# fanliaoooo/xuanpolicy

Measured on AMD Instinct MI355X. Metric: env-steps/sec at num_envs=4096, horizon=128; GAE kernel HBM GB/s vs peak, higher is better.
Workload: dtype f32; 1 GPU; PPO-Clip SynthBox(obs=17,act=6) num_envs=4096/GPU horizon=128, ppo/mujoco.yaml (n_epoch 16, n_minibatch 8, nets [256] LeakyReLU); num_envs_per_gpu=4096, horizon=128, global_envs=4096, minibatch=65536, parallelism=dp1 (one env shard, no collective)

## Files before the change

include/xuanpolicy_amd.h:

```cpp
#ifndef XUANPOLICY_AMD_H
#define XUANPOLICY_AMD_H

#include <stdint.h>

#ifdef __cplusplus
extern "C" {
#endif

typedef struct ihipStream_t *xpa_stream_t;

#define XPA_ABI_VERSION 4
#define XPA_COLSUM_TICKET_INTS 4096

typedef struct {
    int32_t ptr;
    uint32_t step;
    int32_t reserved[2];
} xpa_cursor_t;

enum { XPA_ALGO_PPO = 0, XPA_ALGO_A2C = 1 };
enum { XPA_DIST_GAUSSIAN = 0, XPA_DIST_CATEGORICAL = 1 };

enum {
    XPA_OUT_ACTOR_LOSS = 0,
// ... 332 lines not shown

int xpa_head_gemm_s3_actor(int algo, int dist, int act, int64_t batch, int64_t act_dim, int64_t hidden, const float *x,
                           int64_t ldx, const float *w_hidden, const float *b_hidden, int64_t ld_dz, const float *w,
                           const float *b, float slope, const float *logstd, const int64_t *idx, int64_t n_rows,
                           const float *act_buf, const float *old_logp, const float *adv, const double *adv_partials,
                           int64_t n_adv_partials, float clip_range, float ent_coef, float *dz, float *partial_dw,
                           float *partial_db_hidden, float *partial_db_out, float *loss_partials, int64_t loss_width,
                           xpa_stream_t stream);
int xpa_head_gemm_s3_critic(int act, int64_t batch, int64_t hidden, const float *x, int64_t ldx,
                            const float *w_hidden, const float *b_hidden, int64_t ld_dz, const float *w, const float *b,
                            float slope, const int64_t *idx, int64_t n_rows, const float *ret, float vf_coef, float *dz,
                            float *partial_dw, float *partial_db_hidden, float *partial_db_out, float *loss_partials,
                            int64_t loss_width, xpa_stream_t stream);

int xpa_head_gemm_s3p_actor(int algo, int dist, int act, int64_t batch, int64_t act_dim, int64_t hidden, const float *x,
                            int64_t ldx, const float *w_hidden_split, const float *b_hidden, int64_t ld_dz,
                            const float *w, const float *b, float slope, const float *logstd, const int64_t *idx,
                            int64_t n_rows, const float *act_buf, const float *old_logp, const float *adv,
                            const double *adv_partials, int64_t n_adv_partials, float clip_range, float ent_coef,
                            float *dz, float *partial_dw, float *partial_db_hidden, float *partial_db_out,
                            float *loss_partials, int64_t loss_width, xpa_stream_t stream);
int xpa_head_gemm_s3p_critic(int act, int64_t batch, int64_t hidden, const float *x, int64_t ldx,
                             const float *w_hidden_split, const float *b_hidden, int64_t ld_dz, const float *w,
                             const float *b, float slope, const int64_t *idx, int64_t n_rows, const float *ret,
                             float vf_coef, float *dz, float *partial_dw, float *partial_db_hidden,
                             float *partial_db_out, float *loss_partials, int64_t loss_width, xpa_stream_t stream);
int xpa_head_gemm_s3q_actor(int algo, int dist, int act, int64_t batch, int64_t act_dim, int64_t hidden, const float *x,
                            int64_t ldx, const float *w_hidden_split, const float *b_hidden, int64_t ld_dz,
                            const float *w, const float *b, float slope, const float *logstd, const int64_t *idx,
                            int64_t n_rows, const float *act_buf, const float *old_logp, const float *adv,
                            const double *adv_partials, int64_t n_adv_partials, float clip_range, float ent_coef,
                            float *dz, float *partial_dw, float *partial_db_hidden, float *partial_db_out,
                            float *loss_partials, int64_t loss_width, xpa_stream_t stream);
int xpa_head_gemm_s3q_critic(int act, int64_t batch, int64_t hidden, const float *x, int64_t ldx,
                             const float *w_hidden_split, const float *b_hidden, int64_t ld_dz, const float *w,
                             const float *b, float slope, const int64_t *idx, int64_t n_rows, const float *ret,
                             float vf_coef, float *dz, float *partial_dw, float *partial_db_hidden,
                             float *partial_db_out, float *loss_partials, int64_t loss_width, xpa_stream_t stream);

int xpa_head_gemm_trunk_actor(int algo, int dist, int act, int64_t batch, int64_t act_dim, int64_t hidden,
                              const float *x_rows, int64_t ld_rows, int64_t d_in, const float *w_in, const float *b_in,
                              float slope_in, float *h_out, int64_t ld_h, const float *w_hidden, const float *b_hidden,
                              int64_t ld_dz, const float *w, const float *b, float slope, const float *logstd,
                              const int64_t *idx, int64_t n_rows, const float *act_buf, const float *old_logp,
                              const float *adv, const double *adv_partials, int64_t n_adv_partials, float clip_range,
                              float ent_coef, float *dz, float *partial_dw, float *partial_db_hidden,
                              float *partial_db_out, float *loss_partials, int64_t loss_width, xpa_stream_t stream);
int xpa_head_gemm_trunk_critic(int act, int64_t batch, int64_t hidden, const float *x_rows, int64_t ld_rows,
                               int64_t d_in, const float *w_in, const float *b_in, float slope_in, float *h_out,
                               int64_t ld_h, const float *w_hidden, const float *b_hidden, int64_t ld_dz, const float *w,
                               const float *b, float slope, const int64_t *idx, int64_t n_rows, const float *ret,
                               float vf_coef, float *dz, float *partial_dw, float *partial_db_hidden,
                               float *partial_db_out, float *loss_partials, int64_t loss_width, xpa_stream_t stream);

int64_t xpa_s3_split_bytes(int64_t k, int64_t n);
int xpa_s3_probe(int mask);
int xpa_s3_split_b(const float *b, int64_t k, int64_t n, int64_t sk, int64_t sn, void *out, xpa_stream_t stream);
int xpa_s3_split_batch(int n_mat, const float *const *b, const int64_t *k, const int64_t *sk, const int64_t *sn,
                       void *const *out, xpa_stream_t stream);
int xpa_s3_gemm(const float *a, int64_t lda, const void *b_split, float *c, int64_t ldc, int64_t m, int64_t k, int64_t n,
                xpa_stream_t stream);
int xpa_s3_gemm_group(int n, const float *const *a, const void *const *b_split, float *const *c, int64_t lda,
                      int64_t ldc, int64_t m, int64_t k, xpa_stream_t stream);
int64_t xpa_s3_gemm_group_act_num_partials(int n, int64_t m);
int xpa_s3_gemm_group_act(int n, const float *const *a, const void *const *b_split, float *const *c,
                          const float *const *y, int64_t lda, int64_t ldc, int64_t m, int64_t k, int act, float slope,
                          int64_t channels, float *bias_partial, xpa_stream_t stream);
int64_t xpa_s3_wgrad_num_slices(int64_t rows, int64_t m);
int64_t xpa_s3_gemm_trunk_bwd_num_partials(int64_t rows);
int xpa_s3_gemm_trunk_bwd(const float *dz, int64_t ldz, const void *b_split, int64_t k, const float *h, int64_t ldh,
                          const float *x, int64_t ldx, int64_t rows, int64_t d_in, int act, float slope,
                          float *partial_dw, float *partial_db, xpa_stream_t stream);
int xpa_s3_wgrad(const float *a, int64_t lda, const float *b, int64_t ldb, int64_t rows, int64_t m, int64_t n,
                 int64_t slices, float *out, xpa_stream_t stream);
int xpa_s3_gemm_trunk_bwd_sign(const float *dz, int64_t ldz, const void *b_split, int64_t k, const unsigned *h_sign,
                               const float *x, int64_t ldx, int64_t rows, int64_t d_in, int act, float slope,
                               float *partial_dw, float *partial_db, xpa_stream_t stream);
int xpa_head_gemm_s3q_critic_mask(int act, int64_t batch, int64_t hidden, const float *x, int64_t ldx,
                                  const float *w_hidden_split, const float *b_hidden, int64_t ld_dz, const float *w,
                                  const float *b, float slope, const int64_t *idx, int64_t n_rows, const float *ret,
                                  float vf_coef, float *dz, float *partial_dw, float *partial_db_hidden,
                                  float *partial_db_out, float *loss_partials, int64_t loss_width, xpa_stream_t stream,
                                  unsigned *mask, float *dv);
int xpa_s3_split_batch_scaled(int n_mat, const float *const *b, const int64_t *k, const int64_t *sk, const int64_t *sn,
                              void *const *out, const float *const *rs_w, const float *rs_a, const int64_t *rs_from,
                              float *cs_out, float cs_slope, xpa_stream_t stream);
int xpa_s3_gemm_trunk_bwd_crit(const float *dz_a, int64_t ldz, const void *b_split, int64_t k_a, int64_t k_c,
                               const unsigned *crit_mask, const float *crit_dv, const float *crit_cs,
                               const unsigned *h_sign, const float *x, int64_t ldx, int64_t rows, int64_t d_in, int act,
                               float slope, float *partial_dw, float *partial_db, xpa_stream_t stream);
int xpa_s3_wgrad_pair_slices(int64_t rows, int64_t *sa, int64_t *sc, int64_t *per_a, int64_t *per_c);
int xpa_s3_wgrad_pair_tune(int sa_target);
int xpa_s3_wgrad_pair(const float *dz_a, int64_t lda, const float *h, int64_t ldb, int64_t rows,
                      const unsigned *crit_mask, const float *crit_dv, const float *crit_wc, float crit_slope,
                      int64_t sa, int64_t per_a, int64_t sc, int64_t per_c, float *out_a, float *out_c,
                      xpa_stream_t stream);
int xpa_rollout_post_deferred_norm_rms(
    int64_t n_envs, int64_t horizon, const float *rew, const uint8_t *term, const uint8_t *trunc, const float *final_obs,
    int64_t ld_final, const float *slot_src, int64_t ld_slot, int64_t obs_dim, float *obs_mean, float *obs_var,
    double *obs_count, float obs_clip, float *boot_norm, int64_t ld_norm, float *slot_obs, int32_t *slot_t,
    int64_t n_slots, int32_t *overflow, xpa_cursor_t *cursor, float *ret_mean, float *ret_var, double *ret_count,
    float *returns, float *buf_rew, float *buf_term, uint8_t *buf_closed, float *buf_boot, float gamma,
    int mask_returns, int use_rewnorm, float rew_range, int atari_lifeloss, double *partials, uint32_t *ticket,
    const float *rms_x, int64_t rms_ld, double *rms_part, xpa_stream_t stream);
int xpa_s3_gemm_bias_act_rows(const float *a, int64_t lda, const int64_t *ridx, const void *b_split, float *c,
                              int64_t ldc, int64_t m, int64_t k, const float *bias, int act, float slope,
                              unsigned *sign_out, xpa_stream_t stream);
int xpa_s3_wgrad_rows(const float *a, int64_t lda, const int64_t *aidx, const float *b, int64_t ldb, int64_t rows,
                      int64_t m, int64_t n, int64_t slices, float *out, xpa_stream_t stream);
int xpa_s3_wgrad_padded(const float *a, int64_t lda, const float *b, int64_t ldb, int64_t rows, int64_t m, int64_t n,
                        int64_t slices, float *out, xpa_stream_t stream);
int xpa_s3_gemm_rows_pair(const float *a, int64_t lda, const void *b0_split, const void *b1_split, const float *bias,
                          float *c, int64_t ldc, int64_t m, xpa_stream_t stream);
int xpa_gather_minibatch_pitched(const int64_t *idx, int64_t batch, int64_t n_rows, const void *obs,
                                 int64_t obs_row_bytes, void *obs_out, int64_t out_row_bytes, const float *adv,
                                 double *adv_partials, int32_t *err, xpa_stream_t stream);
int xpa_s3_split_batch_padded(int n_mat, const float *const *b, const int64_t *k, const int64_t *kv, const int64_t *sk,
                              const int64_t *sn, void *const *out, xpa_stream_t stream);
int xpa_s3_gemm_bias_act(const float *a, int64_t lda, const void *b_split, float *c, int64_t ldc, int64_t m, int64_t k,
                         const float *bias, int act, float slope, unsigned *sign_out, xpa_stream_t stream);
int xpa_s3_gemm_trunk_bwd_dz(const float *dz, int64_t ldz, const void *b_split, int64_t k, const unsigned *h_sign,
                             int64_t rows, int act, float slope, float *dz_out, int64_t ld_out, float *partial_db,
                             xpa_stream_t stream);
int xpa_s3_gemm_trunk_bwd_crit_dz(const float *dz_a, int64_t ldz, const void *b_split, int64_t k_a, int64_t k_c,
                                  const unsigned *crit_mask, const float *crit_dv, const float *crit_cs,
                                  const unsigned *h_sign, int64_t rows, int act, float slope, float *dz_out,
                                  int64_t ld_out, float *partial_db, xpa_stream_t stream);
int xpa_colsum_finalize_batch_map(int n_segs, const float *const *partials, const int64_t *n_partials,
                                  const int64_t *cols, float *const *outs, const int64_t *tmap, double *sq,
                                  int32_t *ticket, int algo, int dist, int64_t batch, int64_t act_dim,
                                  const float *loss_partials, int64_t n_loss_partials, float vf_coef, float ent_coef,
                                  float *scalars, float *d_logstd, xpa_stream_t stream);
int xpa_head_gemm_s3r_actor(int algo, int dist, int act, int64_t batch, int64_t act_dim, int64_t hidden,
                            const float *x_rows, int64_t ld_rows, int64_t d_in, const float *w_in, const float *b_in,
                            float slope_in, float *h_out, int64_t ld_h, unsigned *h_sign, const void *w_hidden,
                            const float *b_hidden, int64_t ld_dz, const float *w, const float *b, float slope,
                            const float *logstd, const int64_t *idx, int64_t n_rows, const float *act_buf,
                            const float *old_logp, const float *adv, const double *adv_partials,
                            int64_t n_adv_partials, float clip_range, float ent_coef, float *dz, float *partial_dw,
                            float *partial_db_hidden, float *partial_db_out, float *loss_partials, int64_t loss_width,
                            xpa_stream_t stream);
int xpa_head_gemm_s3r_critic(int act, int64_t batch, int64_t hidden, const float *x_rows, int64_t ld_rows,
                             int64_t d_in, const float *w_in, const float *b_in, float slope_in, const void *w_hidden,
                             const float *b_hidden, int64_t ld_dz, const float *w, const float *b, float slope,
                             const int64_t *idx, int64_t n_rows, const float *ret, float vf_coef, float *dz,
                             float *partial_dw, float *partial_db_hidden, float *partial_db_out, float *loss_partials,
                             int64_t loss_width, xpa_stream_t stream);

int xpa_per_store(double *sum_tree, double *min_tree, const double *max_priority, int64_t n_envs,
                  int64_t capacity, int64_t ptr, double alpha, xpa_stream_t stream);
int xpa_per_update_priorities(double *sum_tree, double *min_tree, double *max_priority, int *scratch,
                              int64_t n_envs, int64_t capacity, int64_t size, const int64_t *idx,
                              const float *priorities, int64_t batch_per_env, double alpha, int *err,
                              xpa_stream_t stream);
int xpa_per_sample(const double *sum_tree, const double *min_tree, int64_t n_envs, int64_t capacity, int64_t size,
                   int64_t batch_per_env, int64_t n_size, const double *uniforms, uint32_t seed, uint32_t counter,
                   double beta, int wrap_uint8, int64_t *steps, int64_t *flat_index, double *weights, int32_t *err,
                   xpa_stream_t stream);

int xpa_store_column(const void *src, int64_t n, int64_t row_bytes, void *dst, int64_t horizon,
                     const xpa_cursor_t *cursor, xpa_stream_t stream);

int xpa_synthatari_step(int64_t n_envs, int64_t n_actions, const float *act_in, int64_t ld_act, uint32_t seed,
                        int32_t max_episode_steps, uint8_t *stack, uint8_t *final_obs, float *rew, uint8_t *term,
                        uint8_t *trunc, int32_t *ep_step, int32_t *ep_index, int32_t *lives, int32_t *paddle,
                        float *ep_score, float *ep_last_score, int32_t *ep_last_len, int32_t *err,
// ... 120 lines not shown
```

xuanpolicy_amd/csrc/sgemm3.hip:

```cpp
#include "xpa_common.h"
#include "s3_split.h"

namespace {

typedef xpa_f32x16 f32x16;
typedef xpa_bf16x8 bf16x8;
typedef __attribute__((address_space(3))) char lds_char_t;

constexpr int kN = 256;
constexpr int kKC = 16;
constexpr int kBImg = 3 * kN * kKC * 2;
template <int W>
struct S3Geom {
    static constexpr int kRows = 32 * W;
    static constexpr int kAImg = kRows * kKC * 4;
    static constexpr int kStage = kAImg + kBImg;
    static constexpr int kPer = kBImg / 1024 / W;
    static constexpr int kDma = 2 + kPer;
    static_assert(kBImg % (1024 * W) == 0, "B image splits evenly over the waves");
};

__device__ __forceinline__ void glds16(const void *g, unsigned lds_wave_base) {
    asm volatile("s_mov_b32 m0, %1\n\ts_nop 0\n\tglobal_load_lds_dwordx4 %0, off" ::"v"(g), "s"(lds_wave_base)
                 : "memory", "m0");
// ... 1148 lines not shown
        if (t < 256) {
            s_dv[t] = r0 + t < M ? cdv[r0 + t] : 0.f;
            s_cs[t] = ccs[t];
        }
    }
    __syncthreads();
    f32x16 acc[8];
#pragma unroll
    for (int cb = 0; cb < 8; ++cb)
#pragma unroll
        for (int r = 0; r < 16; ++r) acc[cb][r] = 0.f;
    const int N = nca + ncc;
    auto chunk_of = [&](int i) { return i < ncc ? nca + i : i - ncc; };
    auto issue_i = [&](int i) {
        const unsigned st = base + (i % 3) * G::kStage;
        const int c = chunk_of(i);
        const int rr = lane >> 2, p = lane & 3;
        if (i >= ncc) {
            const int q = p ^ ((rr >> 2) & 3);
#pragma unroll
            for (int k = 0; k < 2; ++k) {
                int64_t row = r0 + wave * 32 + k * 16 + rr;
                row = row < M ? row : M - 1;
                glds16(a + row * lda + c * kKC + 4 * q, st + (unsigned)((wave * 32 + k * 16) * kKC * 4));
            }
        }
        const char *bsrc = reinterpret_cast<const char *>(bs) + (int64_t)c * kBImg;
#pragma unroll
        for (int j = 0; j < G::kPer; ++j) {
            const int piece = wave * G::kPer + j;
            glds16(bsrc + piece * 1024 + lane * 16, st + (unsigned)(G::kAImg + piece * 1024));
        }
    };
    auto wait_i = [&](int i) {
        if (i + 1 >= N) asm volatile("s_waitcnt vmcnt(0)\n\ts_barrier" ::: "memory");
        else if (i + 1 >= ncc) asm volatile("s_waitcnt vmcnt(%0)\n\ts_barrier" ::"n"(G::kDma) : "memory");
        else asm volatile("s_waitcnt vmcnt(%0)\n\ts_barrier" ::"n"(G::kPer) : "memory");
    };
    issue_i(0);
    if (N > 1) issue_i(1);
    const int hh = lane >> 5, i32 = lane & 31;
    const unsigned *mrow = s_mask + (wave * 32 + i32) * kCMaskStride;
#pragma unroll 1
    for (int i = 0; i < ncc; ++i) {
        wait_i(i);
        if (i + 2 < N) issue_i(i + 2);
        const unsigned wbits = mrow[i >> 1] >> (16 * (i & 1) + 4 * hh);
        unsigned pk[4];
#pragma unroll
        for (int pj = 0; pj < 4; ++pj) {
            const int j0 = 2 * pj, j1 = 2 * pj + 1;
            const int b0 = j0 < 4 ? j0 : j0 + 4, b1 = j1 < 4 ? j1 : j1 + 4;
            pk[pj] = (((wbits >> b0) & 1u) * 0x3F80u) | ((((wbits >> b1) & 1u) * 0x3F80u) << 16);
        }
        const bf16x8 am = __builtin_bit_cast(bf16x8, make_uint4(pk[0], pk[1], pk[2], pk[3]));
        const bf16x8 *bimg = reinterpret_cast<const bf16x8 *>(lds + (i % 3) * G::kStage + G::kAImg) + lane;
#pragma unroll
        for (int cb = 0; cb < 8; ++cb) {
            acc[cb] = __builtin_amdgcn_mfma_f32_32x32x16_bf16(am, bimg[(16 + cb) * 64], acc[cb], 0, 0, 0);
            acc[cb] = __builtin_amdgcn_mfma_f32_32x32x16_bf16(am, bimg[(8 + cb) * 64], acc[cb], 0, 0, 0);
            acc[cb] = __builtin_amdgcn_mfma_f32_32x32x16_bf16(am, bimg[cb * 64], acc[cb], 0, 0, 0);
        }
    }
    {
        const int col = lane & 31;
#pragma unroll
        for (int r = 0; r < 16; ++r) {
            const float dvr = s_dv[wave * 32 + (r & 3) + 8 * (r >> 2) + 4 * hh];
#pragma unroll
            for (int cb = 0; cb < 8; ++cb) acc[cb][r] = dvr * (acc[cb][r] + s_cs[cb * 32 + col]);
        }
    }
#pragma unroll 1
    for (int i = ncc; i < N; ++i) {
        wait_i(i);
        if (i + 2 < N) issue_i(i + 2);
        chunk<8, 0>(lds + (i % 3) * G::kStage, acc, lane, wave);
    }
    __syncthreads();
    tb_epilogue<ACT, true, DZ>(acc, lds, r0, M, t, lane, wave, nullptr, 0, x, ldx, din, slope, p_dw, p_db, hsign,
                               dz_out, ld_out);
}

constexpr int kWgM = 128;
constexpr int kWgKC = 32;
constexpr int kWgAImg = 3 * 4 * 2 * 1024;
constexpr int kWgBImg = 3 * 8 * 2 * 1024;
constexpr int kWgStage = kWgAImg + kWgBImg;

struct WgUnits {
    float a[8], b0[8], b1[8];
};

__device__ __forceinline__ void wg_load(WgUnits &u, const float *__restrict__ A, int64_t lda, const float *__restrict__ B,
                                        int64_t ldb, int64_t k0, int64_t kend, int ma, int sa, int ha, int nb, int sb) {
#pragma unroll
    for (int j = 0; j < 8; ++j) {
        const int64_t ra = k0 + 16 * sa + kmap(ha, j);
        const int64_t rb0 = k0 + 16 * sb + kmap(0, j), rb1 = k0 + 16 * sb + kmap(1, j);
        const float va = A[min(ra, kend - 1) * lda + ma];
        const float v0 = B[min(rb0, kend - 1) * ldb + nb], v1 = B[min(rb1, kend - 1) * ldb + nb];
        u.a[j] = ra < kend ? va : 0.f;
        u.b0[j] = rb0 < kend ? v0 : 0.f;
        u.b1[j] = rb1 < kend ? v1 : 0.f;
    }
}

__device__ __forceinline__ void wg_put(char *st, const float (&v)[8], int off) {
    bf16x8 h, m, l;
    xpa_split8(make_float4(v[0], v[1], v[2], v[3]), make_float4(v[4], v[5], v[6], v[7]), h, m, l);
    *reinterpret_cast<bf16x8 *>(st + off) = h;
    *reinterpret_cast<bf16x8 *>(st + off + 8 * 1024 * ((off < kWgAImg) ? 1 : 2)) = m;
    *reinterpret_cast<bf16x8 *>(st + off + 16 * 1024 * ((off < kWgAImg) ? 1 : 2)) = l;
}

__device__ __forceinline__ void wg_store(char *st, const WgUnits &u, int ml, int sa, int ha, int nb, int sb) {
    wg_put(st, u.a, (((ml >> 5) * 2 + sa) * 64 + ha * 32 + (ml & 31)) * 16);
    wg_put(st, u.b0, kWgAImg + (((nb >> 5) * 2 + sb) * 64 + (nb & 31)) * 16);
    wg_put(st, u.b1, kWgAImg + (((nb >> 5) * 2 + sb) * 64 + 32 + (nb & 31)) * 16);
}

template <int PROBE>
__device__ __forceinline__ void wg_chunk(const char *st, f32x16 (&acc)[2][2], int lane, int wm, int wn) {
#pragma unroll
    for (int s = 0; s < 2; ++s) {
        bf16x8 ah[2], am[2], al[2], bh[2], bm[2], bl[2];
#pragma unroll
        for (int i = 0; i < 2; ++i) {
            const bf16x8 *pa = reinterpret_cast<const bf16x8 *>(st) + ((2 * wm + i) * 2 + s) * 64 + lane;
            ah[i] = pa[0];
            am[i] = pa[8 * 64];
            al[i] = pa[16 * 64];
            const bf16x8 *pb = reinterpret_cast<const bf16x8 *>(st + kWgAImg) + ((2 * wn + i) * 2 + s) * 64 + lane;
            bh[i] = pb[0];
            bm[i] = pb[16 * 64];
            bl[i] = pb[32 * 64];
        }
        if constexpr ((PROBE & 5) != 0) {
#pragma unroll
            for (int i = 0; i < 2; ++i)
#pragma unroll
                for (int j = 0; j < 2; ++j) {
                    if constexpr ((PROBE & 1) != 0)
                        asm volatile("" ::"v"(ah[i]), "v"(am[i]), "v"(al[i]), "v"(bh[j]), "v"(bm[j]), "v"(bl[j]));
                    else acc[i][j] = __builtin_amdgcn_mfma_f32_32x32x16_bf16(ah[i], bh[j], acc[i][j], 0, 0, 0);
                    if constexpr ((PROBE & 1) == 0) asm volatile("" ::"v"(am[i]), "v"(al[i]), "v"(bm[j]), "v"(bl[j]));
                }
            continue;
        }
#pragma unroll
        for (int i = 0; i < 2; ++i)
#pragma unroll
            for (int j = 0; j < 2; ++j) acc[i][j] = xpa_mfma_s3(ah[i], am[i], al[i], bh[j], bm[j], bl[j], acc[i][j]);
    }
}

template <int PROBE>
__global__ __launch_bounds__(512, 1) void s3_wgrad_kernel(const float *__restrict__ A, int64_t lda,
                                                          const float *__restrict__ B, int64_t ldb, int64_t rows,
                                                          int64_t M, int slices, int64_t slice_rows,
                                                          float *__restrict__ out) {
    __shared__ __attribute__((aligned(16))) char lds[2 * kWgStage];
    const int mtiles = (int)(M / kWgM);
    const int nblk = slices * mtiles;
    int L = blockIdx.x;
    if (nblk % 8 == 0) L = (blockIdx.x & 7) * (nblk >> 3) + (blockIdx.x >> 3);
// ... 910 lines not shown
                                          const float *crit_cs, const unsigned *h_sign, int64_t rows, int act,
                                          float slope, float *dz_out, int64_t ld_out, float *partial_db,
                                          xpa_stream_t stream) {
    if (!dz_a || !b_split || !crit_mask || !crit_dv || !crit_cs || !h_sign || !dz_out || !partial_db || rows <= 0 ||
        k_a <= 0 || k_c <= 0 || k_a % kKC != 0 || k_c % kKC != 0 || k_c > 256 || ldz < k_a || (ldz & 3) ||
        (reinterpret_cast<uintptr_t>(dz_a) & 15) || (reinterpret_cast<uintptr_t>(h_sign) & 15) ||
        (reinterpret_cast<uintptr_t>(crit_mask) & 15) || ld_out < kN || act < 0 || act > 1 ||
        (k_a + k_c) / kKC > (1 << 20))
        return (int)hipErrorInvalidValue;
    const dim3 grid((unsigned)xpa_s3_gemm_trunk_bwd_num_partials(rows)), block(512);
    const __bf16 *bs = static_cast<const __bf16 *>(b_split);
    const int nca = (int)(k_a / kKC), ncc = (int)(k_c / kKC);
    if (act == 0)
        s3_trunk_bwd_crit_kernel<0, true><<<grid, block, 0, stream>>>(dz_a, ldz, bs, rows, nca, ncc, crit_mask,
                                                                       crit_dv, crit_cs, nullptr, 0, 0, slope, nullptr,
                                                                       partial_db, h_sign, dz_out, ld_out);
    else
        s3_trunk_bwd_crit_kernel<1, true><<<grid, block, 0, stream>>>(dz_a, ldz, bs, rows, nca, ncc, crit_mask,
                                                                       crit_dv, crit_cs, nullptr, 0, 0, slope, nullptr,
                                                                       partial_db, h_sign, dz_out, ld_out);
    return xpa_launch_status();
}

namespace {
int gemm_bias_act_impl(const float *a, int64_t lda, const int64_t *ridx, const void *b_split, float *c, int64_t ldc,
                       int64_t m, int64_t k, const float *bias, int act, float slope, unsigned *sign_out,
                       xpa_stream_t stream);
}

XPA_API int xpa_s3_gemm_bias_act(const float *a, int64_t lda, const void *b_split, float *c, int64_t ldc, int64_t m,
                                 int64_t k, const float *bias, int act, float slope, unsigned *sign_out,
                                 xpa_stream_t stream) {
    if (lda < k) return (int)hipErrorInvalidValue;
    return gemm_bias_act_impl(a, lda, nullptr, b_split, c, ldc, m, k, bias, act, slope, sign_out, stream);
}

XPA_API int xpa_s3_gemm_bias_act_rows(const float *a, int64_t lda, const int64_t *ridx, const void *b_split, float *c,
                                      int64_t ldc, int64_t m, int64_t k, const float *bias, int act, float slope,
                                      unsigned *sign_out, xpa_stream_t stream) {
    if (!ridx || lda < 4 || k > lda + kKC) return (int)hipErrorInvalidValue;
    return gemm_bias_act_impl(a, lda, ridx, b_split, c, ldc, m, k, bias, act, slope, sign_out, stream);
}

namespace {
int gemm_bias_act_impl(const float *a, int64_t lda, const int64_t *ridx, const void *b_split, float *c, int64_t ldc,
                       int64_t m, int64_t k, const float *bias, int act, float slope, unsigned *sign_out,
                       xpa_stream_t stream) {
    if (!a || !b_split || !c || !bias || m <= 0 || k <= 0 || k % kKC != 0 || ldc < kN ||
        (reinterpret_cast<uintptr_t>(a) & 15) || (lda & 3) || act < 0 || act > 2 || (sign_out && act == 2) ||
        (reinterpret_cast<uintptr_t>(sign_out) & 15) || k / kKC > (1 << 20))
        return (int)hipErrorInvalidValue;
    const __bf16 *bs = static_cast<const __bf16 *>(b_split);
    const int nch = (int)(k / kKC);
    const dim3 grid((unsigned)((m + 255) / 256)), block(512);
    unsigned char *sg = reinterpret_cast<unsigned char *>(sign_out);
    if (act == 0)
        s3_gemm_kernel<8, 3, 0, 0, 1><<<grid, block, 0, stream>>>(a, lda, bs, c, ldc, m, nch, bias, slope, sg, ridx);
    else if (act == 1)
        s3_gemm_kernel<8, 3, 0, 0, 2><<<grid, block, 0, stream>>>(a, lda, bs, c, ldc, m, nch, bias, slope, sg, ridx);
    else
        s3_gemm_kernel<8, 3, 0, 0, 3><<<grid, block, 0, stream>>>(a, lda, bs, c, ldc, m, nch, bias, slope, nullptr,
                                                                  ridx);
    return xpa_launch_status();
}
}

XPA_API int xpa_s3_gemm_value(const float *a, int64_t lda, const void *b_split, float *v, int64_t m, int64_t k,
                              const float *bias, int act, float slope, const float *w_out, const float *b_out,
                              xpa_stream_t stream) {
    if (!a || !b_split || !v || !bias || !w_out || !b_out || m <= 0 || k <= 0 || k % kKC != 0 || lda < k ||
        (reinterpret_cast<uintptr_t>(a) & 15) || (lda & 3) || act < 0 || act > 2 || k / kKC > (1 << 20) ||
        (m + 63) / 64 > 0x7fffffff)
        return (int)hipErrorInvalidValue;
    const __bf16 *bs = static_cast<const __bf16 *>(b_split);
    const int nch = (int)(k / kKC);
    const dim3 grid((unsigned)((m + 63) / 64)), block(128);
    hipStream_t s = (hipStream_t)stream;
    if (act == 0) s3_gemm_value_kernel<2, 4><<<grid, block, 0, s>>>(a, lda, bs, v, m, nch, bias, slope, w_out, b_out);
    else if (act == 1) s3_gemm_value_kernel<2, 5><<<grid, block, 0, s>>>(a, lda, bs, v, m, nch, bias, slope, w_out, b_out);
    else s3_gemm_value_kernel<2, 6><<<grid, block, 0, s>>>(a, lda, bs, v, m, nch, bias, slope, w_out, b_out);
    return xpa_launch_status();
}

XPA_API int xpa_s3_gemm_rows_pair(const float *a, int64_t lda, const void *b0_split, const void *b1_split,
                                  const float *bias, float *c, int64_t ldc, int64_t m, xpa_stream_t stream) {
    if (!a || !b0_split || !b1_split || !bias || !c || m <= 0 || lda < kN || ldc < 2 * kN || (lda & 3) ||
        (reinterpret_cast<uintptr_t>(a) & 15) || (m + kRRows - 1) / kRRows > 0x7fffffff)
        return (int)hipErrorInvalidValue;
    const dim3 grid((unsigned)((m + kRRows - 1) / kRRows), 4);
    const __bf16 *b0 = static_cast<const __bf16 *>(b0_split), *b1 = static_cast<const __bf16 *>(b1_split);
    if (g_s3_probe & 512)
        s3_gemm_r64_kernel<3, 1><<<grid, dim3(256), 0, stream>>>(a, lda, b0, b1, c, ldc, m, kN / kKC, bias);
    else if (g_s3_probe & 1024)
        s3_gemm_r64_kernel<3, 2><<<grid, dim3(256), 0, stream>>>(a, lda, b0, b1, c, ldc, m, kN / kKC, bias);
    else
        s3_gemm_r64_kernel<2, 4><<<grid, dim3(256), 0, stream>>>(a, lda, b0, b1, c, ldc, m, kN / kKC, bias);
    return xpa_launch_status();
}

XPA_API int xpa_s3_gemm_rows_pair_trunk(int act, const float *x, int64_t ldx, int64_t d_in, const float *w,
                                        const float *b, float slope, const float *mean, const float *var, float clip,
                                        float *xn, int64_t ldn, float *col, int64_t col_ld, const xpa_cursor_t *cursor,
                                        const void *b0_split, const void *b1_split, const float *bias, float *c,
                                        int64_t ldc, int64_t m, xpa_stream_t stream) {
    if (!x || !w || !b || !mean || !var || !xn || !b0_split || !b1_split || !bias || !c || m <= 0 || d_in < 1 ||
        d_in > TrunkW<20>::kSt || act < 0 || act > 2 || ldx < d_in || ldn < d_in || ldc < 2 * kN ||
        (col && (!cursor || col_ld < d_in)) || (m + kRRows - 1) / kRRows > 0x7fffffff)
        return (int)hipErrorInvalidValue;
    const dim3 grid((unsigned)((m + kRRows - 1) / kRRows), 4);
    const __bf16 *b0 = static_cast<const __bf16 *>(b0_split), *b1 = static_cast<const __bf16 *>(b1_split);
    hipStream_t s = (hipStream_t)stream;
    const int din = (int)d_in;
#define XPA_K40T_P(A_, D_, P_)                                                                                        \
    s3_gemm_r64_trunk_kernel<3, 2, A_, D_, P_><<<grid, dim3(256), 0, s>>>(x, ldx, din, w, b, slope, mean, var, clip,  \
                                                                           xn, ldn, col, col_ld, cursor, b0, b1, c, ldc, \
                                                                           m, bias)
    if ((g_s3_probe & 12288) && act == 1 && din > 8) {
        if (g_s3_probe & 4096) XPA_K40T_P(1, 20, 1);
        else XPA_K40T_P(1, 20, 2);
        return xpa_launch_status();
    }
    if (din <= 8) {
        if (act == 0) XPA_K40T_P(0, 8, 0);
        else if (act == 1) XPA_K40T_P(1, 8, 0);
        else XPA_K40T_P(2, 8, 0);
    } else {
        if (act == 0) XPA_K40T_P(0, 20, 0);
        else if (act == 1) XPA_K40T_P(1, 20, 0);
        else XPA_K40T_P(2, 20, 0);
    }
#undef XPA_K40T_P
    return xpa_launch_status();
}

XPA_API int xpa_s3_gemm_group(int n, const float *const *a, const void *const *b_split, float *const *c, int64_t lda,
                              int64_t ldc, int64_t m, int64_t k, xpa_stream_t stream) {
    if (n < 1 || n > kS3Groups || !a || !b_split || !c || m <= 0 || k <= 0 || k % kKC != 0 || lda < k || ldc < kN ||
        (lda & 3) || k / kKC > (1 << 20) || (m + 255) / 256 > 0x7fffffff)
        return (int)hipErrorInvalidValue;
    S3Group g{};
    for (int p = 0; p < n; ++p) {
        if (!a[p] || !b_split[p] || !c[p] || (reinterpret_cast<uintptr_t>(a[p]) & 15)) return (int)hipErrorInvalidValue;
        g.a[p] = a[p];
        g.b[p] = static_cast<const __bf16 *>(b_split[p]);
        g.c[p] = c[p];
    }
    s3_gemm_group_kernel<-1><<<dim3((unsigned)((m + 255) / 256), (unsigned)n), dim3(512), 0, stream>>>(
        g, lda, ldc, m, (int)(k / kKC), S3ActBwd{});
    return xpa_launch_status();
}

XPA_API int64_t xpa_s3_gemm_group_act_num_partials(int n, int64_t m) { return (int64_t)n * ((m + 255) / 256); }

XPA_API int xpa_s3_gemm_group_act(int n, const float *const *a, const void *const *b_split, float *const *c,
                                  const float *const *y, int64_t lda, int64_t ldc, int64_t m, int64_t k, int act,
                                  float slope, int64_t channels, float *bias_partial, xpa_stream_t stream) {
    if (n < 1 || n > kS3Groups || !a || !b_split || !c || !y || !bias_partial || m <= 0 || k <= 0 || k % kKC != 0 ||
        lda < k || ldc < kN || (lda & 3) || k / kKC > (1 << 20) || (m + 255) / 256 > 0x7fffffff || act < 0 || act > 2 ||
        (channels != 32 && channels != 64))
        return (int)hipErrorInvalidValue;
    S3Group g{};
    for (int p = 0; p < n; ++p) {
        if (!a[p] || !b_split[p] || !c[p] || !y[p] || (reinterpret_cast<uintptr_t>(a[p]) & 15))
            return (int)hipErrorInvalidValue;
        g.a[p] = a[p];
        g.b[p] = static_cast<const __bf16 *>(b_split[p]);
// ... 56 lines not shown
```

xuanpolicy_amd/ops.py:

```python
import ctypes

import numpy as np
import torch

from . import _lib
from .small_path import small_close, small_close_args, small_close_batch, small_eval, small_eval_batch

ALGO = {"ppo": 0, "a2c": 1}
DIST = {"gaussian": 0, "categorical": 1}
N_OUT = 6
OUT_KEYS = ("actor-loss", "critic-loss", "entropy", "loss", "clip_ratio", "predict_value")


def lib():
    return _lib.load()


class KernelTimer:

    def __init__(self):
        self.enabled = False
        self.only = None
        self.events = {}
        self.hip_pairs = {}
# ... 801 lines not shown
            inner, valid, ld = (int(v) for v in tmap)
            if (part.dim() != 2 or part.shape[1] % inner or valid > part.shape[1] // inner or out.numel() != inner * valid
                    or not out.is_contiguous() or ld != valid):
                raise ValueError("tmap: partials [G, rows * inner], out contiguous [inner, valid], ld == valid")
        self.items.append((part, out, tmap))

    def flush(self, device=None, sq=None):
        if not self.items:
            loss, self.loss = self.loss, None
            if loss is not None:
                a, d, B, K, lp, vf, ent, sc, dls = loss
                dev = device if device is not None else lp.device
                _lib.call(lib().xpa_policy_loss_finalize_sq, a, d, B, K, _p(lp), lp.shape[0], vf, ent, _p(sc), _p(dls),
                          _p(sq) if sq is not None else None, _stream(dev))
            return None, 0
        key = tuple((p.data_ptr(), p.shape[0], p.shape[1], o.data_ptr(), tm) for p, o, tm in self.items)
        plan = self._plans.get(key)
        if plan is None:
            plan = []
            for i in range(0, len(key), self.MAX_SEGS):
                chunk = key[i:i + self.MAX_SEGS]
                n = len(chunk)
                arrs = ((ctypes.c_void_p * n)(*[c[0] for c in chunk]), (ctypes.c_int64 * n)(*[c[1] for c in chunk]),
                        (ctypes.c_int64 * n)(*[c[2] for c in chunk]), (ctypes.c_void_p * n)(*[c[3] for c in chunk]))
                tiles = int(lib().xpa_colsum_batch_tiles(n, ctypes.cast(arrs[1], ctypes.c_void_p),
                                                         ctypes.cast(arrs[2], ctypes.c_void_p)))
                tmap = None
                if any(c[4] is not None for c in chunk):
                    tmap = (ctypes.c_int64 * (3 * n))(*[v for c in chunk for v in (c[4] or (0, 0, 0))])
                plan.append((n, arrs, [ctypes.cast(a, ctypes.c_void_p) for a in arrs], tiles, tmap))
            self._plans[key] = plan
        dev = device if device is not None else self.items[0][0].device
        s = _stream(dev)
        L = lib()
        total = None
        loss, self.loss = self.loss, None
        one = sq is not None and len(plan) == 1 and plan[0][3] + 2 <= sq.numel()
        if loss is not None and not one:
            a, d, B, K, lp, vf, ent, sc, dls = loss
            _lib.call(L.xpa_policy_loss_finalize_sq, a, d, B, K, _p(lp), lp.shape[0], vf, ent, _p(sc), _p(dls),
                      _p(sq) if sq is not None else None, s)
            loss = None
        if one:
            if self._ticket is None:
                self._ticket = torch.zeros((_lib.COLSUM_TICKET_INTS,), dtype=torch.int32, device=dev)
            n, _keep, args, tiles, tmap = plan[0]
            if tmap is not None:
                la = loss if loss is not None else (0, 0, 0, 0, None, 0.0, 0.0, None, None)
                a, d, B, K, lp, vf, ent, sc, dls = la
                _lib.call(L.xpa_colsum_finalize_batch_map, n, *args, ctypes.cast(tmap, ctypes.c_void_p), _p(sq),
                          _p(self._ticket), a, d, B, K, _p(lp) if lp is not None else None,
                          lp.shape[0] if lp is not None else 0, vf, ent, _p(sc) if sc is not None else None,
                          _p(dls) if dls is not None else None, s)
            elif loss is not None:
                a, d, B, K, lp, vf, ent, sc, dls = loss
                _lib.call(L.xpa_colsum_finalize_batch_sq_loss, n, *args, _p(sq), _p(self._ticket), a, d, B, K, _p(lp),
                          lp.shape[0], vf, ent, _p(sc), _p(dls), s)
            else:
                _lib.call(L.xpa_colsum_finalize_batch_sq, n, *args, _p(sq), _p(self._ticket), s)
            total = sq[1 + tiles:2 + tiles]
        else:
            for n, _keep, args, _tiles, tmap in plan:
                if tmap is not None:
                    _lib.call(L.xpa_colsum_finalize_batch_map, n, *args, ctypes.cast(tmap, ctypes.c_void_p), None, None,
                              0, 0, 0, 0, None, 0, 0.0, 0.0, None, None, s)
                else:
                    _lib.call(L.xpa_colsum_finalize_batch, n, *args, s)
        written = sum(o.numel() for _, o, _ in self.items)
        self.items = []
        return total, written


K16W_ENABLED = False
S3_GEMMS = True
S3_HEADS = "s3q"


HEAD_FORMS = {
    "K12": ("xpa_head_fused_actor", "xpa_head_fused_critic"),
    "K16": ("xpa_head_gemm_actor", "xpa_head_gemm_critic"),
    "K16S": ("xpa_head_gemm_s3_actor", "xpa_head_gemm_s3_critic"),
    "K16P": ("xpa_head_gemm_s3p_actor", "xpa_head_gemm_s3p_critic"),
    "K16Q": ("xpa_head_gemm_s3q_actor", "xpa_head_gemm_s3q_critic"),
    "K16Q-mask": ("xpa_head_gemm_s3q_actor", "xpa_head_gemm_s3q_critic_mask"),
    "K16W": ("xpa_head_gemm_ws_actor", "xpa_head_gemm_ws_critic"),
    "K16S+W": ("xpa_head_gemm_s3_actor", "xpa_head_gemm_ws_critic"),
    "K16+W": ("xpa_head_gemm_actor", "xpa_head_gemm_ws_critic"),
    "K16X": ("xpa_head_gemm_trunk_actor", "xpa_head_gemm_critic"),
    "K16R": ("xpa_head_gemm_s3r_actor", "xpa_head_gemm_s3r_critic"),
}


def head_form(gemm, trunk, wh_split, crit_mask, K):
    if not gemm:
        form = "K12"
    elif trunk:
        form = "K16R" if wh_split else "K16X"
    elif K16W_ENABLED:
        form = "K16W" if K <= 8 else "K16S+W" if S3_GEMMS else "K16+W"
    elif wh_split:
        form = "K16Q" if S3_HEADS == "s3q" else "K16P"
    else:
        form = "K16S" if S3_GEMMS else "K16"
    if crit_mask:
        if form != "K16Q":
            raise ValueError("crit_mask needs the K16Q heads")
        form = "K16Q-mask"
    return form


def fused_heads(algo, dist, ws, z_actor, w_actor, b_actor, act_actor, z_critic, w_critic, b_critic, act_critic,
                logstd, act, adv, ret, old_logp=None, idx=None, adv_partials=None, clip_range=0.2, vf_coef=0.25,
                ent_coef=0.0, grads=None, colsum_queue=None, gemm=None, sq_logstd=None, defer_loss=False, trunk=None,
                wh_split=None, crit_mask=None, form=None):
    if algo not in ALGO or dist not in DIST:
        raise ValueError("algo must be ppo|a2c and dist gaussian|categorical")
    H = HEAD_HIDDEN
    B = gemm[0].shape[0] if gemm is not None else z_actor.shape[0]
    K = w_actor.shape[0]
    if ws.batch != B or ws.k != K:
        raise ValueError("fused heads need a matching workspace")
    ld = ws.dz_actor.stride(0)
    if gemm is not None:
        x, (wha, bha), (whc, bhc) = gemm
        _req(x, "x", torch.float32, contiguous=False)
        if tuple(x.shape) != (B, H) or x.stride(1) != 1:
            raise ValueError("x must be [%d, %d] with unit column stride" % (B, H))
        for name, w_ in (("w_h_actor", wha), ("w_h_critic", whc)):
            _req(w_, name, torch.float32, (H, H))
    else:
        for name, zz in (("z_actor", z_actor), ("z_critic", z_critic)):
            _req(zz, name, torch.float32, contiguous=False)
            if tuple(zz.shape) != (B, H) or zz.stride() != (ld, 1):
                raise ValueError("%s must be [%d, %d] with row stride %d" % (name, B, H, ld))
    _req(w_actor, "w_actor", torch.float32, (K, H))
    _req(w_critic, "w_critic", torch.float32, (1, H))
    if idx is not None:
        _req(idx, "idx", torch.int64, (B,))
    rows = adv.numel()
    _req(adv, "adv", torch.float32)
    _req(ret, "ret", torch.float32, (rows,))
    _req(act, "act", torch.float32)
    if act.numel() != rows * (K if dist == "gaussian" else 1):
        raise ValueError("act has %d elements, expected %d" % (act.numel(), rows * (K if dist == "gaussian" else 1)))
    if algo == "ppo":
        _req(old_logp, "old_logp", torch.float32, (rows,))
    if adv_partials is not None:
        _req(adv_partials, "adv_partials", torch.float64)
    dev = w_actor.device
    s = _stream(dev)
    L = lib()
    W = ws.loss_partials.shape[1]
    ev = TIMER.start("heads")
    n_adv = adv_partials.shape[0] if adv_partials is not None else 0
    p_logstd = _p(logstd) if dist == "gaussian" else None
    p_old = _p(old_logp) if algo == "ppo" else None
    if trunk is not None:
        if gemm is None or trunk[4] is not x:
            raise ValueError("trunk needs gemm with x = the trunk's h output")
        xr, w0, b0, slope0, h_out = trunk[:5]
        h_sign = trunk[5] if len(trunk) > 5 else None
        _req(xr, "x_rows", torch.float32)
        din = xr.shape[1]
        if xr.dim() != 2 or xr.shape[0] != B or din > TRUNK_DMAX or tuple(w0.shape) != (H, din):
            raise ValueError("trunk rows must be [%d, <= %d] with w_in [%d, d_in]" % (B, TRUNK_DMAX, H))
    head_a, head_c = (ALGO[algo], DIST[dist], act_actor[0], B, K, H), (act_critic[0], B, H)
    tail_a = (_p(w_actor), _p(b_actor), float(act_actor[1]), p_logstd, _p(idx), rows, _p(act), p_old, _p(adv),
# ... 444 lines not shown
```

Baseline: 10.73 million env-steps/s.

## Add fused 512-thread critic head kernel with GEMM, loss, mask and partial reductions

Adds a new critic-head kernel that runs the hidden-layer GEMM through the triple-buffered LDS pipeline. In its epilogue it applies LeakyReLU, the output projection, the value loss, the sign-mask and dv writes, and block-level reductions of weight and bias gradient partials. The dispatcher uses it when the shapes fit (hidden=256, LeakyReLU, no dz output) and falls back to the previous s3q critic-mask path otherwise. The goal is to cut launches and intermediate memory traffic in the critic backward. The cost is one block per CU with a large LDS footprint and extra code for zeroing unused partial slots.

```diff
diff --git a/include/xuanpolicy_amd.h b/include/xuanpolicy_amd.h
--- a/include/xuanpolicy_amd.h
+++ b/include/xuanpolicy_amd.h
@@ -438,6 +438,13 @@
                                   float vf_coef, float *dz, float *partial_dw, float *partial_db_hidden,
                                   float *partial_db_out, float *loss_partials, int64_t loss_width, xpa_stream_t stream,
                                   unsigned *mask, float *dv);
+int xpa_s3_head_critic_mask(int act, int64_t batch, int64_t hidden, const float *x, int64_t ldx,
+                            const float *w_hidden_split, const float *b_hidden, int64_t ld_dz, const float *w,
+                            const float *b, float slope, const int64_t *idx, int64_t n_rows, const float *ret,
+                            float vf_coef, float *dz, float *partial_dw, float *partial_db_hidden,
+                            float *partial_db_out, float *loss_partials, int64_t loss_width, xpa_stream_t stream,
+                            unsigned *mask, float *dv);
+int xpa_head_critic_form(int form);
 int xpa_s3_split_batch_scaled(int n_mat, const float *const *b, const int64_t *k, const int64_t *sk, const int64_t *sn,
                               void *const *out, const float *const *rs_w, const float *rs_a, const int64_t *rs_from,
                               float *cs_out, float cs_slope, xpa_stream_t stream);
diff --git a/xuanpolicy_amd/csrc/sgemm3.hip b/xuanpolicy_amd/csrc/sgemm3.hip
--- a/xuanpolicy_amd/csrc/sgemm3.hip
+++ b/xuanpolicy_amd/csrc/sgemm3.hip
@@ -1254,6 +1254,167 @@
                                dz_out, ld_out);
 }
 
+__device__ __forceinline__ float hc_row_loss(float v, float retv, bool ok, float vf_coef, float inv_b, float &sum0,
+                                             float &sum1, float &dbo) {
+#pragma clang fp contract(off)
+    const float diff = v - retv;
+    const float dvr = ok ? vf_coef * 2.0f * diff * inv_b : 0.f;
+    sum0 += ok ? diff * diff : 0.f;
+    sum1 += ok ? v : 0.f;
+    dbo += dvr;
+    return dvr;
+}
+
+__global__ __launch_bounds__(512, 1) void s3_head_critic_kernel(
+    const float *__restrict__ a, int64_t lda, const __bf16 *__restrict__ bs, int64_t M, const float *__restrict__ bh,
+    const float *__restrict__ wo, const float *__restrict__ bo, float slope, const int64_t *__restrict__ idx,
+    int64_t n_rows, const float *__restrict__ ret, float vf_coef, float *__restrict__ p_dw, float *__restrict__ p_dbh,
+    float *__restrict__ p_dbo, float *__restrict__ p_loss, int loss_width, int64_t G, unsigned *__restrict__ mask,
+    float *__restrict__ dv) {
+    using Gm = S3Geom<8>;
+    constexpr int kNch = kN / kKC;
+    __shared__ __attribute__((aligned(16))) char lds[3 * Gm::kStage];
+    const unsigned base = __builtin_amdgcn_readfirstlane((unsigned)(uintptr_t)(lds_char_t *)lds);
+    const int t = threadIdx.x, lane = t & 63;
+    const int wave = __builtin_amdgcn_readfirstlane(t >> 6);
+    const int64_t blk = blockIdx.x, r0 = blk * Gm::kRows;
+    f32x16 acc[8];
+#pragma unroll
+    for (int cb = 0; cb < 8; ++cb)
+#pragma unroll
+        for (int r = 0; r < 16; ++r) acc[cb][r] = 0.f;
+    const float *ar[2];
+    {
+        const int rr = lane >> 2, p = lane & 3;
+        const int q = p ^ ((rr >> 2) & 3);
+#pragma unroll
+        for (int i = 0; i < 2; ++i) {
+            int64_t row = r0 + wave * 32 + i * 16 + rr;
+            row = row < M ? row : M - 1;
+            ar[i] = a + row * lda + 4 * q;
+        }
+    }
+    issue_rows<8>(base, ar[0], ar[1], bs, 0, lane, wave);
+    issue_rows<8>(base + Gm::kStage, ar[0], ar[1], bs, 1, lane, wave);
+    float retv = 0.f, okf = 0.f;
+    if (t < Gm::kRows && r0 + t < M) {
+        const int64_t row = idx ? idx[r0 + t] : r0 + t;
+        if (row >= 0 && row < n_rows) {
+            retv = ret[row];
+            okf = 1.f;
+        }
+    }
+    asm volatile("" ::"v"(retv), "v"(okf));
+#pragma unroll 1
+    for (int ch = 0; ch < kNch; ++ch) {
+        if (ch + 1 < kNch) asm volatile("s_waitcnt vmcnt(%0)\n\ts_barrier" ::"n"(Gm::kDma) : "memory");
+        else asm volatile("s_waitcnt vmcnt(0)\n\ts_barrier" ::: "memory");
+        if (ch + 2 < kNch) issue_rows<8>(base + ((ch + 2) % 3) * Gm::kStage, ar[0], ar[1], bs, ch + 2, lane, wave);
+        chunk<8, 0>(lds + (ch % 3) * Gm::kStage, acc, lane, wave);
+    }
+    __syncthreads();
+    float *s_ret = reinterpret_cast<float *>(lds);
+    float *s_ok = s_ret + 256;
+    float *s_dw = s_ok + 256;
+    float *s_dbh = s_dw + 8 * 256;
+    float *s_sc = s_dbh + 8 * 256;
+    if (t < Gm::kRows) {
+        s_ret[t] = retv;
+        s_ok[t] = okf;
+    }
+    __syncthreads();
+    const int h = lane >> 5, col = lane & 31;
+    float bv[8], wv[8], dwc[8], dbc[8];
+#pragma unroll
+    for (int cb = 0; cb < 8; ++cb) {
+        bv[cb] = bh[cb * 32 + col];
+        wv[cb] = wo[cb * 32 + col];
+        dwc[cb] = dbc[cb] = 0.f;
+    }
+    const float b_out = bo[0], inv_b = 1.0f / (float)M;
+    float sum0 = 0.f, sum1 = 0.f, dbo = 0.f;
+#pragma unroll
+    for (int r = 0; r < 16; ++r) {
+        const int rl = wave * 32 + (r & 3) + 8 * (r >> 2) + 4 * h;
+        const int64_t row = r0 + rl;
+        float p = 0.f;
+        unsigned mw = 0u;
+#pragma unroll
+        for (int cb = 0; cb < 8; ++cb) {
+            const float z = acc[cb][r] + bv[cb];
+            const float av = z > 0.f ? z : z * slope;
+            acc[cb][r] = av;
+            const unsigned long long bl = __ballot(av > 0.f);
+            const unsigned wbits = h ? (unsigned)(bl >> 32) : (unsigned)bl;
+            mw = col == cb ? wbits : mw;
+            p = fmaf(av, wv[cb], p);
+        }
+#pragma unroll
+        for (int o = 16; o > 0; o >>= 1) p += __shfl_xor(p, o, 64);
+        const float dvr = hc_row_loss(p + b_out, s_ret[rl], s_ok[rl] != 0.f, vf_coef, inv_b, sum0, sum1, dbo);
+        if (row < M) {
+            if (col < 8) mask[row * 8 + col] = mw;
+            if (col == 8) dv[row] = dvr;
+        }
+#pragma unroll
+        for (int cb = 0; cb < 8; ++cb) {
+            const float av = acc[cb][r];
+            dwc[cb] = fmaf(dvr, av, dwc[cb]);
+            dbc[cb] += (dvr * wv[cb]) * (av > 0.f ? 1.f : slope);
+        }
+        __builtin_amdgcn_sched_barrier(0);
+    }
+#pragma unroll
+    for (int cb = 0; cb < 8; ++cb) {
+        dwc[cb] += __shfl_xor(dwc[cb], 32, 64);
+        dbc[cb] += __shfl_xor(dbc[cb], 32, 64);
+        if (h == 0) {
+            s_dw[wave * 256 + cb * 32 + col] = dwc[cb];
+            s_dbh[wave * 256 + cb * 32 + col] = dbc[cb];
+        }
+    }
+    sum0 += __shfl_xor(sum0, 32, 64);
+    sum1 += __shfl_xor(sum1, 32, 64);
+    dbo += __shfl_xor(dbo, 32, 64);
+    if (lane == 0) {
+        s_sc[wave * 3] = sum0;
+        s_sc[wave * 3 + 1] = sum1;
+        s_sc[wave * 3 + 2] = dbo;
+    }
+    __syncthreads();
+    const int64_t nblk = gridDim.x;
+    if (t < 256) {
+        float sw = s_dw[t], sb = s_dbh[t];
+#pragma unroll
+        for (int w = 1; w < 8; ++w) {
+            sw += s_dw[w * 256 + t];
+            sb += s_dbh[w * 256 + t];
+        }
+        p_dw[blk * 256 + t] = sw;
+        p_dbh[blk * 256 + t] = sb;
+        for (int64_t zb = blk + nblk; zb < G; zb += nblk) {
+            p_dw[zb * 256 + t] = 0.f;
+            p_dbh[zb * 256 + t] = 0.f;
+        }
+    } else if (t == 256) {
+        float s0 = s_sc[0], s1 = s_sc[1], s2 = s_sc[2];
+#pragma unroll
+        for (int w = 1; w < 8; ++w) {
+            s0 += s_sc[w * 3];
+            s1 += s_sc[w * 3 + 1];
+            s2 += s_sc[w * 3 + 2];
+        }
+        p_loss[blk * loss_width + 1] = s0;
+        p_loss[blk * loss_width + 4] = s1;
+        p_dbo[blk] = s2;
+        for (int64_t zb = blk + nblk; zb < G; zb += nblk) {
+            p_loss[zb * loss_width + 1] = 0.f;
+            p_loss[zb * loss_width + 4] = 0.f;
+            p_dbo[zb] = 0.f;
+        }
+    }
+}
+
 constexpr int kWgM = 128;
 constexpr int kWgKC = 32;
 constexpr int kWgAImg = 3 * 4 * 2 * 1024;
@@ -2330,6 +2491,40 @@
     return xpa_launch_status();
 }
 
+namespace {
+int g_head_critic_form = 1;
+}
+XPA_API int xpa_head_critic_form(int form) {
+    const int prev = g_head_critic_form;
+    if (form >= 0) g_head_critic_form = form != 0 ? 1 : 0;
+    return prev;
+}
+
+XPA_API int xpa_s3_head_critic_mask(int act, int64_t batch, int64_t hidden, const float *x, int64_t ldx,
+                                    const float *w_hidden_split, const float *b_hidden, int64_t ld_dz, const float *w,
+                                    const float *b, float slope, const int64_t *idx, int64_t n_rows, const float *ret,
+                                    float vf_coef, float *dz, float *partial_dw, float *partial_db_hidden,
+                                    float *partial_db_out, float *loss_partials, int64_t loss_width, xpa_stream_t stream,
+                                    unsigned *mask, float *dv) {
+    const int64_t nblk = batch > 0 ? (batch + 255) / 256 : 0;
+    const bool args_ok = batch > 0 && x && w_hidden_split && b_hidden && w && b && ret && partial_dw &&
+                         partial_db_hidden && partial_db_out && loss_partials && loss_width >= 5 &&
+                         loss_width <= 0x7fffffff && n_rows > 0 && (idx || n_rows >= batch) && ldx >= kN &&
+                         (ldx & 3) == 0 && ld_dz >= kN;
+    const bool k40h = g_head_critic_form == 1 && args_ok && hidden == kN && act == 1 && !dz && mask && dv &&
+                      ((reinterpret_cast<uintptr_t>(x) | reinterpret_cast<uintptr_t>(w_hidden_split)) & 15) == 0 &&
+                      (reinterpret_cast<uintptr_t>(mask) & 3) == 0 && nblk <= xpa_head_fused_num_partials(batch);
+    if (!k40h)
+        return xpa_head_gemm_s3q_critic_mask(act, batch, hidden, x, ldx, w_hidden_split, b_hidden, ld_dz, w, b, slope,
+                                             idx, n_rows, ret, vf_coef, dz, partial_dw, partial_db_hidden,
+                                             partial_db_out, loss_partials, loss_width, stream, mask, dv);
+    s3_head_critic_kernel<<<dim3((unsigned)nblk), dim3(512), 0, (hipStream_t)stream>>>(
+        x, ldx, reinterpret_cast<const __bf16 *>(w_hidden_split), batch, b_hidden, w, b, slope, idx, n_rows, ret, vf_coef,
+        partial_dw, partial_db_hidden, partial_db_out, loss_partials, (int)loss_width,
+        xpa_head_fused_num_partials(batch), mask, dv);
+    return xpa_launch_status();
+}
+
 XPA_API int xpa_s3_gemm_rows_pair(const float *a, int64_t lda, const void *b0_split, const void *b1_split,
                                   const float *bias, float *c, int64_t ldc, int64_t m, xpa_stream_t stream) {
     if (!a || !b0_split || !b1_split || !bias || !c || m <= 0 || lda < kN || ldc < 2 * kN || (lda & 3) ||
diff --git a/xuanpolicy_amd/ops.py b/xuanpolicy_amd/ops.py
--- a/xuanpolicy_amd/ops.py
+++ b/xuanpolicy_amd/ops.py
@@ -907,7 +907,7 @@
     "K16S": ("xpa_head_gemm_s3_actor", "xpa_head_gemm_s3_critic"),
     "K16P": ("xpa_head_gemm_s3p_actor", "xpa_head_gemm_s3p_critic"),
     "K16Q": ("xpa_head_gemm_s3q_actor", "xpa_head_gemm_s3q_critic"),
-    "K16Q-mask": ("xpa_head_gemm_s3q_actor", "xpa_head_gemm_s3q_critic_mask"),
+    "K16Q-mask": ("xpa_head_gemm_s3q_actor", "xpa_s3_head_critic_mask"),
     "K16W": ("xpa_head_gemm_ws_actor", "xpa_head_gemm_ws_critic"),
     "K16S+W": ("xpa_head_gemm_s3_actor", "xpa_head_gemm_ws_critic"),
     "K16+W": ("xpa_head_gemm_actor", "xpa_head_gemm_ws_critic"),
```

After: 11.04 million env-steps/s (median of 6 runs). +2.8%, better.
